# pierrenodet/spark-ensemble

Measured on AMD Instinct MI355X. Metric: rows/sec (whole node) GBMClassifier 100 trees depth=8 at 1/2/4/8 MI355X, higher is better.
Workload: dtype fp32; 1 GPU; model=GBMClassifier(bernoulli, 265 trees, depth=8, bins=256), global_batch=10000000, rows_per_gpu=10000000, features=256, parallelism=dp1

## Files before the change

### csrc/common.h

```cpp
#pragma once

#include <torch/extension.h>
#include <hip/hip_runtime.h>

#include <cstdint>

#define CHECK_GPU(x) TORCH_CHECK(x.is_cuda(), #x " must be on GPU")
#define CHECK_CONTIG(x) TORCH_CHECK(x.is_contiguous(), #x " must be contiguous")

inline int64_t ceil_div(int64_t a, int64_t b) { return (a + b - 1) / b; }

__device__ inline unsigned f32_sortable(float f) {
  unsigned u = __float_as_uint(f);
  return (u & 0x80000000u) ? ~u : (u | 0x80000000u);
}
__device__ inline float sortable_f32(unsigned s) {
  unsigned u = (s & 0x80000000u) ? (s & 0x7FFFFFFFu) : ~s;
  return __uint_as_float(u);
}

enum UploadSlot : int {
  kSlotHistChunks = 0,
  kSlotHistNodes = 1,
  kSlotPartCursors = 2,
  kSlotPartChunks = 3,
  kSlotPartSegStart = 4,
  kSlotGatherSegs = 5,
  kSlotLeafSegs = kSlotGatherSegs,
  kSlotLeafTree = 6,
  kSlotLeafVal = 7,
  kSlotClassChunks = 8,
  kSlotClassNodes = 9,
  kUploadSlots = 12,
};

torch::Tensor h2d_async(const void* src, size_t bytes, UploadSlot slot,
                        const torch::Device& dev);

void launch_hist_decode(float* out, const long long* stage, const int* nodes,
                        const float* scales, int n_multi, int64_t FBC, int C,
                        hipStream_t stream);

void split_argmax_wide(torch::Tensor gain, torch::Tensor feat,
                       torch::Tensor bin, torch::Tensor left_stats,
                       torch::Tensor hist, int D, double lam,
                       double min_child_weight, double min_instances,
                       double min_info_gain);
int64_t hist_build_class(torch::Tensor out, torch::Tensor bins,
                         torch::Tensor bins_t, torch::Tensor label,
                         torch::Tensor weight, torch::Tensor row_idx,
                         torch::Tensor node_offsets, torch::Tensor node_col0,
                         int64_t num_bins, int64_t num_classes, int64_t nn,
                         double w_max, bool identity_rows);

void forest_contrib(torch::Tensor out, torch::Tensor x, torch::Tensor ranges,
                    torch::Tensor path_off, torch::Tensor path_m,
                    torch::Tensor path_v, torch::Tensor e_feat,
                    torch::Tensor e_lo, torch::Tensor e_hi, torch::Tensor e_z,
                    int64_t rows_per_tile, double scale);

void logreg_loss_grad(torch::Tensor payload, torch::Tensor x, torch::Tensor y,
                      torch::Tensor w, torch::Tensor wmat, bool has_bias);
bool logreg_fused_supported(int64_t F, int64_t K);
```

### csrc/ops.hip

```cpp

#include <ATen/hip/HIPContext.h>

#include <chrono>
#include <cstring>
#include <tuple>
#include <vector>

#include "common.h"
#include "hist_plan.h"

torch::Tensor h2d_async(const void* src, size_t bytes, UploadSlot slot,
                        const torch::Device& dev) {
  static thread_local torch::Tensor pin[2 * kUploadSlots];
  static thread_local hipEvent_t done[2 * kUploadSlots] = {};
  static thread_local unsigned char flip[kUploadSlots] = {};
  flip[slot] ^= 1;
  const int bi = slot * 2 + flip[slot];
  auto& b = pin[bi];
  if (done[bi]) (void)hipEventSynchronize(done[bi]);
  if (!b.defined() || (size_t)b.numel() < bytes) {
    size_t cap = 4096;
    while (cap < bytes) cap *= 2;
    b = torch::empty({(int64_t)cap},
                     torch::TensorOptions().dtype(torch::kByte)
// ... 605 lines not shown
    base_l = atomicAdd(cursors + node * 2 + 0, tot);
    base_r = atomicAdd(cursors + node * 2 + 1, -(len - tot)) - (len - tot);
    loc_l = 0;
    loc_r = 0;
  }
  __syncthreads();

  for (int i = threadIdx.x; i < ((len + 63) & ~63); i += blockDim.x) {
    const bool active = i < len;
    const unsigned long long word = bits[i >> 6];
    const bool left = (word >> lane) & 1ull;
    const unsigned long long lmask = word;
    const unsigned long long rmask = __ballot(active) & ~word;
    int lbase = 0, rbase = 0;
    if (lane == 0) {
      lbase = atomicAdd(&loc_l, (int)__popcll(lmask));
      rbase = atomicAdd(&loc_r, (int)__popcll(rmask));
    }
    lbase = __shfl(lbase, 0, 64);
    rbase = __shfl(rbase, 0, 64);
    if (active) {
      const int r = row_idx[start + i];
      if (left) {
        const int pos = base_l + lbase + (int)__popcll(lmask & ((1ull << lane) - 1ull));
        new_rows[pos] = r;
      } else {
        const int pos = base_r + rbase + (int)__popcll(rmask & ((1ull << lane) - 1ull));
        new_rows[pos] = r;
      }
    }
  }
}

void partition_rows(torch::Tensor new_rows, torch::Tensor left_counts,
                    torch::Tensor bins, torch::Tensor bins_t,
                    torch::Tensor row_idx,
                    torch::Tensor node_offsets, torch::Tensor feat,
                    torch::Tensor thr) {
  auto tpA = std::chrono::steady_clock::now();
  CHECK_GPU(new_rows); CHECK_GPU(bins); CHECK_GPU(row_idx);
  CHECK_GPU(feat); CHECK_GPU(thr); CHECK_GPU(left_counts);
  const int F = (int)bins.size(1);
  const int n_nodes = (int)node_offsets.numel() - 1;
  auto offs = node_offsets.accessor<int64_t, 1>();

  std::vector<int> cur_v(n_nodes * 2);
  std::vector<int> chunk_v;
  int64_t total_rows = offs[n_nodes];
  int64_t chunk_rows =
      std::max<int64_t>(8192, ceil_div(total_rows, (int64_t)2048));
  chunk_rows = std::min<int64_t>(chunk_rows, 65536);
  for (int nd = 0; nd < n_nodes; ++nd) {
    cur_v[nd * 2 + 0] = (int)offs[nd];
    cur_v[nd * 2 + 1] = (int)offs[nd + 1];
    for (int64_t c = offs[nd]; c < offs[nd + 1]; c += chunk_rows) {
      chunk_v.push_back(nd);
      chunk_v.push_back((int)c);
      chunk_v.push_back((int)std::min<int64_t>(chunk_rows, offs[nd + 1] - c));
    }
  }
  auto stream = at::hip::getCurrentHIPStream();
  static const bool part_dbg = getenv("SEA_PART_DEBUG") != nullptr;
  auto tp0 = std::chrono::steady_clock::now();
  auto cursors_b = h2d_async(cur_v.data(), cur_v.size() * 4,
                             kSlotPartCursors, bins.device());
  auto cursors = cursors_b.view(torch::kInt32);
  auto tp1 = std::chrono::steady_clock::now();
  if (!chunk_v.empty()) {
    auto chunks_b = h2d_async(chunk_v.data(), chunk_v.size() * 4, kSlotPartChunks,
                              bins.device());
    auto chunks = chunks_b.view(torch::kInt32);
    auto tp2 = std::chrono::steady_clock::now();
    const int n_chunks = (int)(chunk_v.size() / 3);
    const size_t bit_lds = (size_t)((chunk_rows + 63) / 64) * 8;
    const uint8_t* bt_ptr =
        bins_t.defined() && bins_t.numel() ? bins_t.data_ptr<uint8_t>()
                                           : nullptr;
    hipLaunchKernelGGL(partition_kernel, dim3(n_chunks), dim3(256), bit_lds,
                       stream,
                       new_rows.data_ptr<int>(), cursors.data_ptr<int>(),
                       bins.data_ptr<uint8_t>(), bt_ptr,
                       row_idx.data_ptr<int>(),
                       chunks.data_ptr<int>(), feat.data_ptr<int>(),
                       thr.data_ptr<int>(), F, (long long)bins.size(0));
    if (part_dbg) {
      auto tp3 = std::chrono::steady_clock::now();
      auto us = [](auto a, auto b) {
        return std::chrono::duration_cast<std::chrono::microseconds>(b - a)
            .count();
      };
      fprintf(stderr,
              "[part c++] entry=%ldus cursors=%ldus chunks=%ldus launch=%ldus\n",
              (long)us(tpA, tp0), (long)us(tp0, tp1), (long)us(tp1, tp2),
              (long)us(tp2, tp3));
    }
  }
  auto lcur = cursors.view({n_nodes, 2}).select(1, 0);
  std::vector<int> seg_v(n_nodes);
  for (int nd = 0; nd < n_nodes; ++nd) seg_v[nd] = (int)offs[nd];
  auto seg_b = h2d_async(seg_v.data(), seg_v.size() * 4, kSlotPartSegStart,
                         bins.device());
  auto seg_start = seg_b.view(torch::kInt32);
  left_counts.copy_(lcur - seg_start);
}


__global__ void tree_predict_kernel(float* __restrict__ out,
                                    const float* __restrict__ x,
                                    const int* __restrict__ feat,
                                    const float* __restrict__ thr,
                                    const int* __restrict__ left,
                                    const float* __restrict__ leaf,
                                    int64_t n, int F, int D) {
  int64_t i = blockIdx.x * (int64_t)blockDim.x + threadIdx.x;
  int64_t stride = gridDim.x * (int64_t)blockDim.x;
  for (; i < n; i += stride) {
    const float* xr = x + i * F;
    int node = 0;
    int f = feat[0];
    while (f >= 0) {
      node = left[node] + (xr[f] <= thr[node] ? 0 : 1);
      f = feat[node];
    }
    const float* lv = leaf + (int64_t)node * D;
    float* o = out + i * D;
    for (int d = 0; d < D; ++d) o[d] = lv[d];
  }
}

void tree_predict(torch::Tensor out, torch::Tensor x, torch::Tensor feat,
                  torch::Tensor thr, torch::Tensor left, torch::Tensor leaf) {
  CHECK_GPU(out); CHECK_GPU(x);
  int64_t n = x.size(0);
  int F = (int)x.size(1);
  int D = (int)leaf.size(1);
  auto stream = at::hip::getCurrentHIPStream();
// ... 699 lines not shown
  TORCH_CHECK(!want_hess || D == 1, "hessian accumulation is scalar-only");
  TORCH_CHECK(payload.numel() >= 1 + D + (want_hess ? 1 : 0), "payload size");
  auto stream = at::hip::getCurrentHIPStream();
  int blocks = (int)std::min<int64_t>(ceil_div(n, 256 * 8), 2048);
  const int width = 2 + D;
  auto partials = torch::empty({(int64_t)blocks * width},
                               payload.options());
#define LS_LAUNCH(DD)                                                         \
  hipLaunchKernelGGL(line_search_eval_kernel<DD>, dim3(blocks), dim3(256), 0, \
                     stream, partials.data_ptr<float>(),                      \
                     label.data_ptr<float>(), pred.data_ptr<float>(),         \
                     dir.data_ptr<float>(), weight.data_ptr<float>(),         \
                     coeff.data_ptr<float>(), n, (int)loss_id, (float)param,  \
                     want_hess ? 1 : 0)
  switch (D) {
    case 1: LS_LAUNCH(1); break;
    case 2: LS_LAUNCH(2); break;
    case 3: LS_LAUNCH(3); break;
    case 4: LS_LAUNCH(4); break;
    case 5: LS_LAUNCH(5); break;
    case 6: LS_LAUNCH(6); break;
    case 7: LS_LAUNCH(7); break;
    case 8: LS_LAUNCH(8); break;
  }
#undef LS_LAUNCH
  const int rthreads = (256 / width) * width;
  hipLaunchKernelGGL(ls_reduce_kernel, dim3(1), dim3(rthreads), 0, stream,
                     payload.data_ptr<float>(), partials.data_ptr<float>(),
                     blocks, width, std::min(width, (int)payload.numel()));
}


template <int C>
__global__ void split_argmax_kernel(
    unsigned long long* __restrict__ best,
    const float* __restrict__ hist,
    int F, int B, int D, float lam, float min_child_weight,
    float min_instances) {
  const int node = blockIdx.x;
  const int f = blockIdx.y * (blockDim.x >> 6) + (threadIdx.x >> 6);
  const int lane = threadIdx.x & 63;
  if (f >= F) return;
  const float* h = hist + (((int64_t)node * F + f) * (int64_t)B) * C;
  const int BPL = (B + 63) >> 6;
  const int idx_c = C - 1;

  float loc[4][C];
  float tot[C];
#pragma unroll
  for (int c = 0; c < C; ++c) tot[c] = 0.0f;
  for (int i = 0; i < BPL; ++i) {
    const int b = lane * BPL + i;
#pragma unroll
    for (int c = 0; c < C; ++c) loc[i][c] = 0.0f;
    if (b < B) {
#pragma unroll
      for (int c = 0; c < C; ++c) {
        loc[i][c] = h[(int64_t)b * C + c];
        tot[c] += loc[i][c];
      }
    }
  }
  float pre[C], parent[C];
#pragma unroll
  for (int c = 0; c < C; ++c) {
    float v = tot[c];
    for (int off = 1; off < 64; off <<= 1) {
      const float u = __shfl_up(v, off, 64);
      if (lane >= off) v += u;
    }
    pre[c] = v - tot[c];
    parent[c] = __shfl(v, 63, 64);
  }
  float pg2 = 0.0f;
#pragma unroll
  for (int d = 0; d < C; ++d)
    if (d < D) pg2 += parent[d] * parent[d];
  const float parent_score = pg2 / (parent[D] + lam);

  float run[C];
#pragma unroll
  for (int c = 0; c < C; ++c) run[c] = pre[c];
  unsigned best_s = 0u;
  int best_b = -1;
  for (int i = 0; i < BPL; ++i) {
    const int b = lane * BPL + i;
    if (b >= B) break;
#pragma unroll
    for (int c = 0; c < C; ++c) run[c] += loc[i][c];
    if (b < B - 1) {
      const float hl = run[D], hr = parent[D] - run[D];
      const float cl = run[idx_c], cr = parent[idx_c] - run[idx_c];
      if (hl >= min_child_weight && hr >= min_child_weight &&
          cl >= min_instances && cr >= min_instances) {
        float gl = 0.0f, gr = 0.0f;
#pragma unroll
        for (int d = 0; d < C; ++d)
          if (d < D) {
            const float l = run[d], r = parent[d] - run[d];
            gl += l * l;
            gr += r * r;
          }
        const float gain =
            gl / (hl + lam) + gr / (hr + lam) - parent_score;
        const unsigned s = f32_sortable(gain);
        if (s > best_s) { best_s = s; best_b = b; }
      }
    }
  }
  for (int off = 32; off > 0; off >>= 1) {
    const unsigned os = __shfl_down(best_s, off, 64);
    const int ob = __shfl_down(best_b, off, 64);
    if (os > best_s) { best_s = os; best_b = ob; }
  }
  if (lane == 0 && best_b >= 0) {
    const unsigned long long packed =
        ((unsigned long long)best_s << 32) | (unsigned)(f * B + best_b);
    atomicMax(&best[node], packed);
  }
}

template <int C>
__global__ void split_decode_kernel(
    float* __restrict__ gain, int* __restrict__ feat, int* __restrict__ bin,
    float* __restrict__ left_stats,
    const unsigned long long* __restrict__ best,
    const float* __restrict__ hist, int F, int B, float min_info_gain) {
  const int node = blockIdx.x;
  const unsigned long long p = best[node];
  const float g = sortable_f32((unsigned)(p >> 32));
  __shared__ float acc[C];
  if (threadIdx.x < C) acc[threadIdx.x] = 0.0f;
  __syncthreads();
  if (p == 0ull || !(g >= min_info_gain)) {
    if (threadIdx.x == 0) {
      gain[node] = -INFINITY;
      feat[node] = -1;
      bin[node] = -1;
    }
    if (threadIdx.x < C) left_stats[node * C + threadIdx.x] = 0.0f;
    return;
  }
  const int fb = (int)(p & 0xFFFFFFFFull);
  const int f = fb / B, b = fb % B;
  const float* h = hist + (((int64_t)node * F + f) * (int64_t)B) * C;
  float part[C];
#pragma unroll
  for (int c = 0; c < C; ++c) part[c] = 0.0f;
  for (int i = threadIdx.x; i <= b; i += blockDim.x)
#pragma unroll
    for (int c = 0; c < C; ++c) part[c] += h[(int64_t)i * C + c];
#pragma unroll
  for (int c = 0; c < C; ++c)
    if (part[c] != 0.0f) atomicAdd(&acc[c], part[c]);
  __syncthreads();
  if (threadIdx.x == 0) {
    gain[node] = g;
    feat[node] = f;
    bin[node] = b;
  }
  if (threadIdx.x < C) left_stats[node * C + threadIdx.x] = acc[threadIdx.x];
}

void split_argmax(torch::Tensor gain, torch::Tensor feat, torch::Tensor bin,
                  torch::Tensor left_stats, torch::Tensor hist, int64_t d_dims,
                  double lam, double min_child_weight, double min_instances,
                  double min_info_gain) {
  CHECK_GPU(hist); CHECK_CONTIG(hist);
  const int n = (int)hist.size(0);
  const int F = (int)hist.size(1);
  const int B = (int)hist.size(2);
  const int C = (int)hist.size(3);
  const int D = d_dims > 0 ? (int)d_dims : C - 2;
  TORCH_CHECK(C >= 2 && C <= 34, "split_argmax: 2 <= C <= 34");
  TORCH_CHECK(B >= 2 && B <= 256, "split_argmax: 2 <= B <= 256");
  TORCH_CHECK(D >= 1 && D < C, "split_argmax: bad D");
  if (C > 8) {
    CHECK_GPU(gain); CHECK_GPU(feat); CHECK_GPU(bin); CHECK_GPU(left_stats);
    split_argmax_wide(gain, feat, bin, left_stats, hist, D, lam,
                      min_child_weight, min_instances, min_info_gain);
    return;
  }
  auto best = torch::zeros({n}, hist.options().dtype(torch::kInt64));
  auto stream = at::hip::getCurrentHIPStream();
  const int fpb = 4;
#define SA_LAUNCH(CC)                                                         \
  do {                                                                        \
    hipLaunchKernelGGL(split_argmax_kernel<CC>,                               \
                       dim3(n, (F + fpb - 1) / fpb), dim3(64 * fpb), 0,       \
                       stream,                                                \
                       (unsigned long long*)best.data_ptr<int64_t>(),         \
                       hist.data_ptr<float>(), F, B, D, (float)lam,           \
                       (float)min_child_weight, (float)min_instances);        \
    hipLaunchKernelGGL(split_decode_kernel<CC>, dim3(n), dim3(64), 0, stream, \
                       gain.data_ptr<float>(), feat.data_ptr<int>(),          \
                       bin.data_ptr<int>(), left_stats.data_ptr<float>(),     \
                       (unsigned long long*)best.data_ptr<int64_t>(),         \
                       hist.data_ptr<float>(), F, B, (float)min_info_gain);   \
  } while (0)
  switch (C) {
    case 2: SA_LAUNCH(2); break;
    case 3: SA_LAUNCH(3); break;
    case 4: SA_LAUNCH(4); break;
    case 5: SA_LAUNCH(5); break;
    case 6: SA_LAUNCH(6); break;
    case 7: SA_LAUNCH(7); break;
    case 8: SA_LAUNCH(8); break;
  }
#undef SA_LAUNCH
}

std::tuple<int64_t, torch::Tensor, torch::Tensor> hist_plan_debug(
    torch::Tensor node_offsets, torch::Tensor node_col0, int64_t row_bound,
    int64_t col_bound, int64_t lds_bytes, int64_t n_groups) {
  auto offs = node_offsets.to(torch::kInt64).contiguous();
  auto col0 = node_col0.to(torch::kInt32).contiguous();
  const int n_nodes = (int)offs.numel() - 1;
  TORCH_CHECK(col0.numel() == 0 || col0.numel() == n_nodes,
              "node_col0 must be empty or have one entry per node");
  HistPlan plan = plan_hist_chunks(
      offs.data_ptr<int64_t>(), n_nodes,
      col0.numel() ? col0.data_ptr<int>() : nullptr, row_bound,
      (int)col_bound, (size_t)lds_bytes, (int)n_groups, 0);
  auto i32 = torch::TensorOptions().dtype(torch::kInt32);
  auto chunks = torch::tensor(plan.table, i32).view({plan.n_chunks, 5});
  auto multi = torch::tensor(plan.multi_nodes, i32);
  return {plan.chunk_rows, chunks, multi};
}

std::tuple<torch::Tensor, torch::Tensor> hist_plan_slots_debug(
    torch::Tensor node_offsets, torch::Tensor node_col0, int64_t row_bound,
    int64_t col_bound, int64_t lds_bytes, int64_t n_groups) {
  auto offs = node_offsets.to(torch::kInt64).contiguous();
  auto col0 = node_col0.to(torch::kInt32).contiguous();
  const int n_nodes = (int)offs.numel() - 1;
  TORCH_CHECK(col0.numel() == 0 || col0.numel() == n_nodes,
              "node_col0 must be empty or have one entry per node");
  HistPlan plan = plan_hist_chunks(
      offs.data_ptr<int64_t>(), n_nodes,
      col0.numel() ? col0.data_ptr<int>() : nullptr, row_bound,
      (int)col_bound, (size_t)lds_bytes, (int)n_groups, 0);
  auto i32 = torch::TensorOptions().dtype(torch::kInt32);
  return {torch::tensor(plan.slot_first, i32),
          torch::tensor(plan.slot_count, i32)};
}

PYBIND11_MODULE(TORCH_EXTENSION_NAME, m) {
  m.def("_hist_plan", &hist_plan_debug,
        "host-side chunk plan of the histogram kernels (no device)");
  m.def("_hist_plan_slots", &hist_plan_slots_debug,
        "first record and record count of each staging slot of _hist_plan");
  m.def("gather_ranges_gh", &gather_ranges_gh,
        "gather_ranges plus the compact gh rows of the gathered rows");
  m.def("logreg_loss_grad", &logreg_loss_grad,
        "single-pass fused logistic loss+gradient");
  m.def("logreg_fused_supported", &logreg_fused_supported);
  m.def("split_argmax", &split_argmax,
        "fused best-split gain scan + argmax over node histograms");
  m.def("sample_weights", &sample_weights, "counter-based Poisson/Bernoulli row weights");
  m.def("bin_features", &bin_features, "quantile binning f32 -> u8");
  m.def("hist_build", &hist_build, "LDS-staged node histograms",
        py::arg("out"), py::arg("bins"), py::arg("gh"), py::arg("row_idx"),
        py::arg("node_offsets"), py::arg("num_bins"), py::arg("d_dims"),
        py::arg("max_abs"), py::arg("identity_rows"), py::arg("node_col0"),
        py::arg("c_per_node"), py::arg("gh_by_position") = false);
  m.def("hist_build_class", &hist_build_class,
        "label-indexed node histograms for K-class gini trees");
  m.def("partition_rows", &partition_rows, "block-aggregated node partition");
  m.def("tree_predict", &tree_predict, "single-tree batched predict");
  m.def("forest_predict", &forest_predict, "packed-forest weighted predict");
  m.def("forest_predict2", &forest_predict2,
        "LDS-staged tree-group-tiled forest predict");
  m.def("forest_contrib", &forest_contrib,
        "per-row feature contributions (TreeSHAP) of a packed forest");
  m.def("transpose_u8", &transpose_u8, "tiled u8 matrix transpose");
  m.def("gather_ranges", &gather_ranges,
        "one-pass concat of contiguous index ranges");
  m.def("leaf_scatter", &leaf_scatter,
        "scatter per-segment leaf values into the [N, T] train-pred matrix");
  m.def("grad_hess", &grad_hess, "fused per-row loss gradient/hessian");
  m.def("line_search_eval", &line_search_eval, "fused loss+grad line-search payload");
  m.def("newton_chain_1d", &newton_chain_1d,
        "device-chained safeguarded-Newton stage-weight search");
}
```

### spark_ensemble_amd/models/tree_grower.py

```python

from __future__ import annotations

from dataclasses import dataclass
from typing import Dict, List, Optional, Tuple

import torch

from ..ops import dispatch as ops
from ..parallel import Comm


@dataclass
class GrowParams:
    max_depth: int = 5
    max_bins: int = 32
    min_instances_per_node: int = 1
    min_info_gain: float = 0.0
    min_child_weight: float = 0.0
    lam: float = 1e-6


def ensure_binned(frame, x: torch.Tensor, max_bins: int):
    cached = frame.cache_get("bins", x, max_bins) if frame is not None else None
    if cached is not None:
# ... 580 lines not shown
        cnt_col = torch.tensor([float(v) for v in root_lens], device=device)
    if root_tot_in is None:
        cols = [g_sum, h_sum.unsqueeze(1)]
        if NN == 2:
            cols.append(cnt_col.unsqueeze(1))
        root_tot = torch.cat(cols, dim=1)
        if comm is not None:
            comm.all_reduce_(root_tot)
        totals = root_tot.cpu()

    covers_t[:, 0] = totals[:, D]

    node_tree = torch.arange(T, dtype=torch.long)
    node_nid = torch.zeros(T, dtype=torch.long)
    off_acc = [0]
    for v in root_lens:
        off_acc.append(off_acc[-1] + v)
    offsets = torch.tensor(off_acc, dtype=torch.int64)
    hists: Optional[torch.Tensor] = None
    parent_of_t: Optional[torch.Tensor] = None
    built_mask_t: Optional[torch.Tensor] = None

    edges_cpu = edges.cpu()
    idx_c = C - 1

    capture = train_pred_out is not None and D == 1
    tp_arena = (
        torch.zeros(N, T, dtype=torch.float32, device=device)
        if capture else None
    )

    pending_writes = None

    def _finalize_and_capture(idx_t, offs, ridx):
        if idx_t.numel() == 0:
            return
        t_ids = node_tree[idx_t]
        nids = node_nid[idx_t]
        g = totals[idx_t, :D]
        h = totals[idx_t, D]
        denom = (h + params.lam).unsqueeze(1)
        vals = torch.where(denom > 0, g / denom, torch.zeros_like(g))
        leaves_t[t_ids, nids] = vals
        if capture:
            starts = offs[idx_t]
            lens = offs[idx_t + 1] - starts
            nz = (lens > 0).nonzero(as_tuple=True)[0]
            if nz.numel():
                ops.leaf_scatter(tp_arena, ridx, starts[nz], lens[nz],
                                 t_ids[nz], vals[nz, 0])

    for depth in range(params.max_depth + 1):
        n_active = int(node_tree.numel())
        if n_active == 0:
            break
        if depth == params.max_depth:
            _finalize_and_capture(torch.arange(n_active), offsets, row_idx)
            break

        split_args = dict(
            lam=params.lam,
            min_child_weight=params.min_child_weight,
            min_instances=params.min_instances_per_node,
            min_info_gain=params.min_info_gain,
            d_dims=D,
        )
        lvl_mask = None
        if feature_masks is not None:
            lvl_mask = feature_masks.index_select(
                0, _to_dev_async(node_tree, device)
            )
        if hists is None:
            if class_mode:
                new_h = _class_hist(row_idx, offsets, node_tree,
                                    identity=(root_rows is None and T == 1))
            else:
                new_h = ops.hist_build_forest(
                    bins, gh, row_idx, offsets,
                    (node_tree * C).to(torch.int32), B, C, gh_max, d_dims=D,
                )
            hists, gain, feat, b, left_stats = _finish_level_split(
                new_h, None, None, None, None, None, n_active, (F, B, C),
                device, comm, split_args, split_mask=lvl_mask,
            )
        else:
            built_cpu = built_mask_t.nonzero(as_tuple=True)[0]
            nb_cpu = (~built_mask_t).nonzero(as_tuple=True)[0]
            bh = None
            if built_cpu.numel():
                starts = offsets[built_cpu]
                lens = offsets[built_cpu + 1] - starts
                b_off = torch.zeros(built_cpu.numel() + 1, dtype=torch.int64)
                b_off[1:] = torch.cumsum(lens, 0)
                if class_mode:
                    build_rows = ops.gather_ranges(row_idx, starts, lens)
                    bh = _class_hist(build_rows, b_off, node_tree[built_cpu])
                else:
                    build_rows, gh_b = ops.gather_ranges_gh(
                        row_idx, gh, starts, lens, node_tree[built_cpu] * C,
                        C,
                    )
                    bh = ops.hist_build_forest(
                        bins, gh_b, build_rows, b_off,
                        torch.zeros(built_cpu.numel(), dtype=torch.int32),
                        B, C, gh_max, d_dims=D, gh_by_position=True,
                    )
            hists, gain, feat, b, left_stats = _finish_level_split(
                bh, _to_dev_async(built_cpu, device), hists,
                _to_dev_async(nb_cpu, device),
                _to_dev_async(nb_cpu ^ 1, device),
                _to_dev_async(parent_of_t[nb_cpu], device), n_active,
                (F, B, C), device, comm, split_args, split_mask=lvl_mask,
            )
        pack_d = torch.cat([
            gain, feat.to(torch.float32), b.to(torch.float32),
            left_stats.reshape(-1),
        ])
        ev = None
        if bins.is_cuda:
            pack_h = torch.empty(pack_d.numel(), dtype=torch.float32,
                                 pin_memory=True)
            pack_h.copy_(pack_d, non_blocking=True)
            ev = torch.cuda.Event()
            ev.record()

        pr_async = None
        if bins.is_cuda:
            pr_async = ops.partition_rows_async(bins, row_idx, offsets, feat, b)

        if pending_writes is not None:
            pending_writes()
            pending_writes = None

        if ev is not None:
            ev.synchronize()
            pack = pack_h
        else:
            pack = pack_d
        gain_cpu = pack[:n_active]
        feat_cpu = pack[n_active:2 * n_active].to(torch.int32)
        b_cpu = pack[2 * n_active:3 * n_active].to(torch.int32)
        left_stats = pack[3 * n_active:].reshape(n_active, C)

        do_split = torch.isfinite(gain_cpu)
        ns_idx = (~do_split).nonzero(as_tuple=True)[0]
        _finalize_and_capture(ns_idx, offsets, row_idx)
        if not bool(do_split.any()):
            break

        s_idx = do_split.nonzero(as_tuple=True)[0]
        t_ids = node_tree[s_idx]
        nids = node_nid[s_idx]
        f_l = feat_cpu[s_idx].long()
        b_l = b_cpu[s_idx].long()
        counts = torch.bincount(t_ids, minlength=T)
        firsts = torch.cumsum(counts, 0) - counts
        rank = torch.arange(s_idx.numel(), dtype=torch.long) - firsts[t_ids]
        cid = cur_len[t_ids] + 2 * rank
        cur_len += 2 * counts

        hists = hists.index_select(0, _to_dev_async(s_idx, device))

        l_st = left_stats[s_idx]
        r_st = totals[s_idx] - l_st
        totals = torch.stack([l_st, r_st], dim=1).reshape(-1, C)
        l_cnt = l_st[:, idx_c]
        r_cnt = r_st[:, idx_c]
        built_mask_t = torch.stack([l_cnt <= r_cnt, l_cnt > r_cnt],
                                   dim=1).reshape(-1)
        parent_of_t = torch.arange(s_idx.numel(),
                                   dtype=torch.long).repeat_interleave(2)
        node_tree = t_ids.repeat_interleave(2)
        node_nid = torch.stack([cid, cid + 1], dim=1).reshape(-1)

        def _writes(t_ids=t_ids, nids=nids, f_l=f_l, b_l=b_l,
                    gains=gain_cpu[s_idx].double(), cid=cid,
                    l_cov=l_st[:, D], r_cov=r_st[:, D]):
            feats_t[t_ids, nids] = f_l.to(torch.int32)
            thrs_t[t_ids, nids] = edges_cpu[f_l, b_l]
            fi.index_put_((t_ids, f_l), gains, accumulate=True)
            lefts_t[t_ids, nids] = cid.to(torch.int32)
            covers_t[t_ids, cid] = l_cov
            covers_t[t_ids, cid + 1] = r_cov
        pending_writes = _writes

        if pr_async is not None:
            new_rows, new_offs, _ = ops.partition_rows_finish(*pr_async)
        else:
            split_feat = torch.where(do_split, feat_cpu,
                                     torch.full_like(feat_cpu, -1))
            new_rows, new_offs, _ = ops.partition_rows(
                bins, row_idx, offsets,
                split_feat.to(torch.int32), b_cpu.to(torch.int32),
            )
# ... 48 lines not shown
```

### spark_ensemble_amd/ops/dispatch.py

```python

from __future__ import annotations

import math
import os
from typing import Optional

import torch

from . import reference

_hip = None
_hip_error: Optional[str] = None


def _load_hip():
    global _hip, _hip_error
    if _hip is not None or _hip_error is not None:
        return _hip
    try:
        from . import hip_ext

        _hip = hip_ext.load()
    except Exception as e:
        _hip_error = f"{type(e).__name__}: {e}"
# ... 80 lines not shown
                    )
                    parts.append(part[..., :w])
                    if ci == len(spans) - 1:
                        parts.append(part[..., w:])
                return torch.cat(parts, dim=-1)
            return _hist_build_launch(
                m, bins, gh, row_idx, node_offsets, _EMPTY_I32, num_bins, C,
                max_abs, d_dims, identity_rows,
            )
    return reference.hist_build(bins, gh, row_idx, node_offsets, num_bins)


_EMPTY_I32 = torch.empty(0, dtype=torch.int32)
_EMPTY_U8 = torch.empty(0, dtype=torch.uint8)


def _hist_build_launch(m, bins, gh, row_idx, node_offsets, node_col0,
                       num_bins, c_per_node, max_abs, d_dims, identity_rows,
                       gh_by_position=False):
    out = torch.empty(
        node_offsets.numel() - 1, bins.shape[1], num_bins, c_per_node,
        dtype=torch.float32, device=bins.device,
    )
    m.hist_build(
        out, bins, gh.contiguous(), row_idx.to(torch.int32),
        node_offsets.to(torch.int64).cpu().contiguous(), int(num_bins),
        int(d_dims), max_abs.to(torch.float32), bool(identity_rows),
        node_col0, int(c_per_node), bool(gh_by_position),
    )
    return out


def hist_build_forest(bins, gh, row_idx, node_offsets, node_col0, num_bins,
                      c_per_node, max_abs, d_dims=1, gh_by_position=False):
    if bins.is_cuda:
        m = _require_hip("hist_build")
        if m is not None:
            return _hist_build_launch(
                m, bins, gh, row_idx, node_offsets,
                node_col0.to(torch.int32).cpu().contiguous(), num_bins,
                c_per_node, max_abs, d_dims, False, gh_by_position,
            )
    if gh_by_position:
        pos = torch.arange(row_idx.numel(), device=row_idx.device)
        return reference.hist_build_forest(
            bins.index_select(0, row_idx.long()), gh, pos, node_offsets,
            node_col0, num_bins, c_per_node
        )
    return reference.hist_build_forest(
        bins, gh, row_idx, node_offsets, node_col0, num_bins, c_per_node
    )


last_hist_build_class_info: dict = {}


def hist_build_class(bins, label, weight, row_idx, node_offsets, node_col0,
                     num_bins, num_classes, nn, w_max=None,
                     identity_rows=False, transposed=None):
    if bins.is_cuda:
        m = _require_hip("hist_build_class")
        if m is not None:
            n_nodes = node_offsets.numel() - 1
            F = bins.shape[1]
            C = int(num_classes) + int(nn)
            if w_max is None:
                w_max = float(weight.max()) if weight.numel() else 1.0
            if transposed is None:
                transposed = os.environ.get("SEA_CLASS_HIST_SRC") != "rowmajor"
            bt = _bins_transposed(bins) if transposed else _EMPTY_U8
            out = torch.empty(n_nodes, F, num_bins, C, dtype=torch.float32,
                              device=bins.device)
            n_multi = m.hist_build_class(
                out, bins, bt, label, weight.contiguous(),
# ... 8 lines not shown
    return reference.hist_build_class(
        bins, label, weight, row_idx, node_offsets, node_col0, num_bins,
        num_classes, nn,
    )


SPLIT_WIDE_MAX_C = 34


def split_search(hist, lam=1e-6, min_child_weight=0.0, min_instances=1.0, min_info_gain=0.0, d_dims=-1):
    if hist.is_cuda:
        c_chk = hist.shape[3]
        if c_chk > SPLIT_WIDE_MAX_C:
            return reference.split_search(
                hist, lam, min_child_weight, min_instances, min_info_gain,
                d_dims,
            )
        m = _require_hip("split_argmax")
        if m is not None:
            n, f, b, c = hist.shape
            gain = torch.empty(n, dtype=torch.float32, device=hist.device)
            feat = torch.empty(n, dtype=torch.int32, device=hist.device)
            bin_ = torch.empty(n, dtype=torch.int32, device=hist.device)
            left_stats = torch.empty(n, c, dtype=torch.float32, device=hist.device)
            m.split_argmax(
                gain, feat, bin_, left_stats, hist.contiguous(),
                int(d_dims), float(lam), float(min_child_weight),
                float(min_instances), float(min_info_gain),
            )
            return gain, feat.long(), bin_.long(), left_stats
    return reference.split_search(hist, lam, min_child_weight, min_instances, min_info_gain, d_dims)


def partition_rows(bins, row_idx, node_offsets, feat, thr):
    if bins.is_cuda:
        m = _require_hip("partition_rows")
        if m is not None:
            new_rows, lc_dev, offs_cpu = partition_rows_async(
                bins, row_idx, node_offsets, feat, thr
            )
            return partition_rows_finish(new_rows, lc_dev, offs_cpu)
    return reference.partition_rows(bins, row_idx, node_offsets, feat, thr)


_BT_CACHE: list = []


def _bins_transposed(bins):
    import weakref

    m = _load_hip()
    if m is None or not bins.is_cuda:
        return None
    _BT_CACHE[:] = [(w, b) for (w, b) in _BT_CACHE if w() is not None]
    for wr, bt in _BT_CACHE:
        if wr() is bins:
            return bt
    n, f = bins.shape
    bt = torch.empty(f, n, dtype=torch.uint8, device=bins.device)
    m.transpose_u8(bt, bins)
    _BT_CACHE.insert(0, (weakref.ref(bins), bt))
    del _BT_CACHE[1:]
    return bt


def partition_rows_async(bins, row_idx, node_offsets, feat, thr):
    import time as _time

    _prof = os.environ.get("SEA_GROW_PROF") == "1"
    _t0 = _time.perf_counter() if _prof else 0.0
    m = _require_hip("partition_rows")
    n = node_offsets.numel() - 1
    offs_cpu = node_offsets.to(torch.int64).cpu()
    row_idx = row_idx.to(torch.int32)
    new_rows = torch.empty_like(row_idx)
    left_counts = torch.zeros(n, dtype=torch.int32, device=bins.device)
    f32 = feat.to(torch.int32).to(bins.device)
    t32 = thr.to(torch.int32).to(bins.device)
    if _prof:
        _t1 = _time.perf_counter()
    bt = _bins_transposed(bins)
    m.partition_rows(
        new_rows,
        left_counts,
        bins,
        bt if bt is not None else _EMPTY_U8,
        row_idx,
        offs_cpu,
        f32,
        t32,
    )
    lc_h = torch.empty(left_counts.numel(), dtype=torch.int32,
                       pin_memory=True)
    lc_h.copy_(left_counts, non_blocking=True)
    ev = torch.cuda.Event()
    ev.record()
    if _prof:
        _t2 = _time.perf_counter()
        print(f"[part prof] prep={(_t1-_t0)*1000:.2f} native={(_t2-_t1)*1000:.2f}")
    return new_rows, (lc_h, ev), offs_cpu


def gather_ranges(src, starts, lens):
    if src.is_cuda:
        m = _require_hip("gather_ranges")
        if m is not None:
            out = torch.empty(int(lens.sum()), dtype=torch.int32,
                              device=src.device)
            m.gather_ranges(out, src, starts.to(torch.int64),
                            lens.to(torch.int64))
            return out
    st, ln = starts.tolist(), lens.tolist()
    segs = [src[s:s + l] for s, l in zip(st, ln) if l > 0]
    if not segs:
# ... 15 lines not shown
                               col0.to(torch.int64))
            return out, gh_out
    rows = gather_ranges(src, starts, lens)
    segs = [
        gh[src[s:s + l].long(), c0:c0 + C]
        for s, l, c0 in zip(starts.tolist(), lens.tolist(), col0.tolist())
        if l > 0
    ]
    if not segs:
        return rows, gh.new_empty(0, C)
    return rows, torch.cat(segs)


def leaf_scatter(tp, row_idx, starts, lens, tree, val):
    if tp.is_cuda:
        m = _require_hip("leaf_scatter")
        if m is not None:
            m.leaf_scatter(tp, row_idx, starts.to(torch.int64),
                           lens.to(torch.int64), tree.to(torch.int64),
                           val.to(torch.float32))
            return
    st, ln = starts.tolist(), lens.tolist()
    tl, vl = tree.tolist(), val.tolist()
    for s, l, t, v in zip(st, ln, tl, vl):
        if l > 0:
            tp[row_idx[s:s + l].long(), int(t)] = float(v)


def partition_rows_finish(new_rows, left_counts, offs_cpu):
    n = offs_cpu.numel() - 1
    if isinstance(left_counts, tuple):
        lc_h, ev = left_counts
        ev.synchronize()
        lc = lc_h.to(torch.int64)
    else:
        lc = left_counts.cpu().to(torch.int64)
    sizes = torch.empty(2 * n, dtype=torch.int64)
    seg = offs_cpu[1:] - offs_cpu[:-1]
    sizes[0::2] = lc
    sizes[1::2] = seg - lc
    new_offs = torch.cat([torch.zeros(1, dtype=torch.int64), sizes.cumsum(0)])
    return new_rows, new_offs, lc


def tree_predict(x, feature, threshold, left_child, leaf_value, max_depth):
    if x.is_cuda:
        m = _require_hip("tree_predict")
        if m is not None:
            N = x.shape[0]
            D = leaf_value.shape[1]
            out = torch.empty(N, D, dtype=torch.float32, device=x.device)
            m.tree_predict(
                out,
                x.contiguous(),
                feature.to(torch.int32).to(x.device),
                threshold.to(torch.float32).to(x.device),
                left_child.to(torch.int32).to(x.device),
                leaf_value.to(torch.float32).to(x.device).contiguous(),
            )
            return out
    return reference.tree_predict(x, feature, threshold, left_child, leaf_value, max_depth)


def forest_predict(x, trees, weights=None, max_depth=64, cache=None):
    if x.is_cuda and trees:
        m = _require_hip("forest_predict")
        if m is not None:
# ... 325 lines not shown
```

Baseline: 1.219 billion rows/sec.

## Fuse sibling-subtraction, level histogram assembly and split search into one kernel

Adds a level_split op whose kernel builds each node's histogram (copying built rows or computing parent minus sibling), optionally stores it, and runs the split scan in one pass, then decodes straight into a packed result buffer. This replaces the gather/subtract/index_select steps, the separate split search and the torch.cat packing with fewer launches and fewer passes over the histograms. Partition also returns raw cursors copied to pinned host memory, so the device-side left-count subtraction kernel and its upload disappear. The cost is a host-side table build per level and heavier validation on the host.

```diff
diff --git a/csrc/common.h b/csrc/common.h
--- a/csrc/common.h
+++ b/csrc/common.h
@@ -31,6 +31,7 @@
   kSlotLeafVal = 7,
   kSlotClassChunks = 8,
   kSlotClassNodes = 9,
+  kSlotLevelTable = 10,
   kUploadSlots = 12,
 };
 
diff --git a/csrc/ops.hip b/csrc/ops.hip
--- a/csrc/ops.hip
+++ b/csrc/ops.hip
@@ -661,14 +661,14 @@
   }
 }
 
-void partition_rows(torch::Tensor new_rows, torch::Tensor left_counts,
-                    torch::Tensor bins, torch::Tensor bins_t,
-                    torch::Tensor row_idx,
-                    torch::Tensor node_offsets, torch::Tensor feat,
-                    torch::Tensor thr) {
+static torch::Tensor partition_launch(torch::Tensor new_rows,
+                                      torch::Tensor bins, torch::Tensor bins_t,
+                                      torch::Tensor row_idx,
+                                      torch::Tensor node_offsets,
+                                      torch::Tensor feat, torch::Tensor thr) {
   auto tpA = std::chrono::steady_clock::now();
   CHECK_GPU(new_rows); CHECK_GPU(bins); CHECK_GPU(row_idx);
-  CHECK_GPU(feat); CHECK_GPU(thr); CHECK_GPU(left_counts);
+  CHECK_GPU(feat); CHECK_GPU(thr);
   const int F = (int)bins.size(1);
   const int n_nodes = (int)node_offsets.numel() - 1;
   auto offs = node_offsets.accessor<int64_t, 1>();
@@ -724,13 +724,44 @@
               (long)us(tp2, tp3));
     }
   }
-  auto lcur = cursors.view({n_nodes, 2}).select(1, 0);
+  return cursors.view({n_nodes, 2});
+}
+
+void partition_rows(torch::Tensor new_rows, torch::Tensor left_counts,
+                    torch::Tensor bins, torch::Tensor bins_t,
+                    torch::Tensor row_idx,
+                    torch::Tensor node_offsets, torch::Tensor feat,
+                    torch::Tensor thr) {
+  CHECK_GPU(left_counts);
+  auto cursors = partition_launch(new_rows, bins, bins_t, row_idx,
+                                  node_offsets, feat, thr);
+  const int n_nodes = (int)node_offsets.numel() - 1;
+  auto offs = node_offsets.accessor<int64_t, 1>();
+  auto lcur = cursors.select(1, 0);
   std::vector<int> seg_v(n_nodes);
   for (int nd = 0; nd < n_nodes; ++nd) seg_v[nd] = (int)offs[nd];
   auto seg_b = h2d_async(seg_v.data(), seg_v.size() * 4, kSlotPartSegStart,
                          bins.device());
   auto seg_start = seg_b.view(torch::kInt32);
   left_counts.copy_(lcur - seg_start);
+}
+
+torch::Tensor partition_rows_cursors(torch::Tensor new_rows,
+                                     torch::Tensor bins, torch::Tensor bins_t,
+                                     torch::Tensor row_idx,
+                                     torch::Tensor node_offsets,
+                                     torch::Tensor feat, torch::Tensor thr) {
+  CHECK_CONTIG(new_rows); CHECK_CONTIG(row_idx); CHECK_CONTIG(feat);
+  CHECK_CONTIG(thr);
+  const int64_t n_nodes = node_offsets.numel() - 1;
+  TORCH_CHECK(feat.scalar_type() == torch::kInt32 &&
+                  thr.scalar_type() == torch::kInt32 &&
+                  feat.numel() == n_nodes && thr.numel() == n_nodes,
+              "partition_rows_cursors: feat and thr are int32 [n_nodes]");
+  TORCH_CHECK(new_rows.numel() == row_idx.numel(),
+              "partition_rows_cursors: new_rows must match row_idx");
+  return partition_launch(new_rows, bins, bins_t, row_idx, node_offsets, feat,
+                          thr);
 }
 
 
@@ -1496,6 +1527,72 @@
 
 
 template <int C>
+__device__ __forceinline__ void split_scan_wave(
+    unsigned long long* __restrict__ best, float (&loc)[4][C], float (&tot)[C],
+    int node, int f, int lane, int B, int D, float lam,
+    float min_child_weight, float min_instances) {
+  const int BPL = (B + 63) >> 6;
+  const int idx_c = C - 1;
+  float pre[C], parent[C];
+#pragma unroll
+  for (int c = 0; c < C; ++c) {
+    float v = tot[c];
+    for (int off = 1; off < 64; off <<= 1) {
+      const float u = __shfl_up(v, off, 64);
+      if (lane >= off) v += u;
+    }
+    pre[c] = v - tot[c];
+    parent[c] = __shfl(v, 63, 64);
+  }
+  float pg2 = 0.0f;
+#pragma unroll
+  for (int d = 0; d < C; ++d)
+    if (d < D) pg2 += parent[d] * parent[d];
+  const float parent_score = pg2 / (parent[D] + lam);
+
+  float run[C];
+#pragma unroll
+  for (int c = 0; c < C; ++c) run[c] = pre[c];
+  unsigned best_s = 0u;
+  int best_b = -1;
+  for (int i = 0; i < BPL; ++i) {
+    const int b = lane * BPL + i;
+    if (b >= B) break;
+#pragma unroll
+    for (int c = 0; c < C; ++c) run[c] += loc[i][c];
+    if (b < B - 1) {
+      const float hl = run[D], hr = parent[D] - run[D];
+      const float cl = run[idx_c], cr = parent[idx_c] - run[idx_c];
+      if (hl >= min_child_weight && hr >= min_child_weight &&
+          cl >= min_instances && cr >= min_instances) {
+        float gl = 0.0f, gr = 0.0f;
+#pragma unroll
+        for (int d = 0; d < C; ++d)
+          if (d < D) {
+            const float l = run[d], r = parent[d] - run[d];
+            gl += l * l;
+            gr += r * r;
+          }
+        const float gain =
+            gl / (hl + lam) + gr / (hr + lam) - parent_score;
+        const unsigned s = f32_sortable(gain);
+        if (s > best_s) { best_s = s; best_b = b; }
+      }
+    }
+  }
+  for (int off = 32; off > 0; off >>= 1) {
+    const unsigned os = __shfl_down(best_s, off, 64);
+    const int ob = __shfl_down(best_b, off, 64);
+    if (os > best_s) { best_s = os; best_b = ob; }
+  }
+  if (lane == 0 && best_b >= 0) {
+    const unsigned long long packed =
+        ((unsigned long long)best_s << 32) | (unsigned)(f * B + best_b);
+    atomicMax(&best[node], packed);
+  }
+}
+
+template <int C>
 __global__ void split_argmax_kernel(
     unsigned long long* __restrict__ best,
     const float* __restrict__ hist,
@@ -1507,7 +1604,6 @@
   if (f >= F) return;
   const float* h = hist + (((int64_t)node * F + f) * (int64_t)B) * C;
   const int BPL = (B + 63) >> 6;
-  const int idx_c = C - 1;
 
   float loc[4][C];
   float tot[C];
@@ -1525,66 +1621,57 @@
       }
     }
   }
-  float pre[C], parent[C];
-#pragma unroll
-  for (int c = 0; c < C; ++c) {
-    float v = tot[c];
-    for (int off = 1; off < 64; off <<= 1) {
-      const float u = __shfl_up(v, off, 64);
-      if (lane >= off) v += u;
-    }
-    pre[c] = v - tot[c];
-    parent[c] = __shfl(v, 63, 64);
-  }
-  float pg2 = 0.0f;
-#pragma unroll
-  for (int d = 0; d < C; ++d)
-    if (d < D) pg2 += parent[d] * parent[d];
-  const float parent_score = pg2 / (parent[D] + lam);
-
-  float run[C];
-#pragma unroll
-  for (int c = 0; c < C; ++c) run[c] = pre[c];
-  unsigned best_s = 0u;
-  int best_b = -1;
+  split_scan_wave<C>(best, loc, tot, node, f, lane, B, D, lam,
+                     min_child_weight, min_instances);
+}
+
+template <int C>
+__global__ void level_scan_kernel(
+    unsigned long long* __restrict__ best,
+    float* level,
+    const float* built,
+    const float* __restrict__ parent,
+    const int* __restrict__ tab,
+    int store, int F, int B, int D, float lam, float min_child_weight,
+    float min_instances) {
+  const int node = blockIdx.x;
+  const int f = blockIdx.y * (blockDim.x >> 6) + (threadIdx.x >> 6);
+  const int lane = threadIdx.x & 63;
+  if (f >= F) return;
+  const int b_row = tab[node * 3 + 0];
+  const int64_t slice = (int64_t)B * C;
+  const float* h = built + ((int64_t)(b_row >= 0 ? b_row : tab[node * 3 + 2]) *
+                                F + f) * slice;
+  const float* ph =
+      b_row >= 0 ? nullptr
+                 : parent + ((int64_t)tab[node * 3 + 1] * F + f) * slice;
+  float* o = level + ((int64_t)node * F + f) * slice;
+  const int BPL = (B + 63) >> 6;
+
+  float loc[4][C];
+  float tot[C];
+#pragma unroll
+  for (int c = 0; c < C; ++c) tot[c] = 0.0f;
   for (int i = 0; i < BPL; ++i) {
     const int b = lane * BPL + i;
-    if (b >= B) break;
-#pragma unroll
-    for (int c = 0; c < C; ++c) run[c] += loc[i][c];
-    if (b < B - 1) {
-      const float hl = run[D], hr = parent[D] - run[D];
-      const float cl = run[idx_c], cr = parent[idx_c] - run[idx_c];
-      if (hl >= min_child_weight && hr >= min_child_weight &&
-          cl >= min_instances && cr >= min_instances) {
-        float gl = 0.0f, gr = 0.0f;
-#pragma unroll
-        for (int d = 0; d < C; ++d)
-          if (d < D) {
-            const float l = run[d], r = parent[d] - run[d];
-            gl += l * l;
-            gr += r * r;
-          }
-        const float gain =
-            gl / (hl + lam) + gr / (hr + lam) - parent_score;
-        const unsigned s = f32_sortable(gain);
-        if (s > best_s) { best_s = s; best_b = b; }
-      }
-    }
-  }
-  for (int off = 32; off > 0; off >>= 1) {
-    const unsigned os = __shfl_down(best_s, off, 64);
-    const int ob = __shfl_down(best_b, off, 64);
-    if (os > best_s) { best_s = os; best_b = ob; }
-  }
-  if (lane == 0 && best_b >= 0) {
-    const unsigned long long packed =
-        ((unsigned long long)best_s << 32) | (unsigned)(f * B + best_b);
-    atomicMax(&best[node], packed);
-  }
-}
-
-template <int C>
+#pragma unroll
+    for (int c = 0; c < C; ++c) loc[i][c] = 0.0f;
+    if (b < B) {
+#pragma unroll
+      for (int c = 0; c < C; ++c) {
+        float v = h[(int64_t)b * C + c];
+        if (ph) v = ph[(int64_t)b * C + c] - v;
+        if (store) o[(int64_t)b * C + c] = v;
+        loc[i][c] = v;
+        tot[c] += loc[i][c];
+      }
+    }
+  }
+  split_scan_wave<C>(best, loc, tot, node, f, lane, B, D, lam,
+                     min_child_weight, min_instances);
+}
+
+template <int C, bool PACK = false>
 __global__ void split_decode_kernel(
     float* __restrict__ gain, int* __restrict__ feat, int* __restrict__ bin,
     float* __restrict__ left_stats,
@@ -1601,6 +1688,10 @@
       gain[node] = -INFINITY;
       feat[node] = -1;
       bin[node] = -1;
+      if (PACK) {
+        gain[gridDim.x + node] = -1.0f;
+        gain[2 * gridDim.x + node] = -1.0f;
+      }
     }
     if (threadIdx.x < C) left_stats[node * C + threadIdx.x] = 0.0f;
     return;
@@ -1622,6 +1713,10 @@
     gain[node] = g;
     feat[node] = f;
     bin[node] = b;
+    if (PACK) {
+      gain[gridDim.x + node] = (float)f;
+      gain[2 * gridDim.x + node] = (float)b;
+    }
   }
   if (threadIdx.x < C) left_stats[node * C + threadIdx.x] = acc[threadIdx.x];
 }
@@ -1674,6 +1769,135 @@
 #undef SA_LAUNCH
 }
 
+void level_split(torch::Tensor level, torch::Tensor pack, torch::Tensor feat,
+                 torch::Tensor bin, torch::Tensor built, torch::Tensor parent,
+                 torch::Tensor table, int64_t d_dims, double lam,
+                 double min_child_weight, double min_instances,
+                 double min_info_gain) {
+  CHECK_GPU(level); CHECK_GPU(pack); CHECK_GPU(feat); CHECK_GPU(bin);
+  CHECK_GPU(built);
+  CHECK_CONTIG(level); CHECK_CONTIG(pack); CHECK_CONTIG(feat);
+  CHECK_CONTIG(bin); CHECK_CONTIG(built); CHECK_CONTIG(parent);
+  CHECK_CONTIG(table);
+  TORCH_CHECK(!table.is_cuda() && table.scalar_type() == torch::kInt32 &&
+                  table.dim() == 2 && table.size(1) == 3,
+              "level_split: table must be a host int32 [n, 3]");
+  TORCH_CHECK(level.dim() == 4 && built.dim() == 4,
+              "level_split: level and built must be [n, F, B, C]");
+  TORCH_CHECK(level.scalar_type() == torch::kFloat32 &&
+                  built.scalar_type() == torch::kFloat32 &&
+                  pack.scalar_type() == torch::kFloat32 &&
+                  feat.scalar_type() == torch::kInt32 &&
+                  bin.scalar_type() == torch::kInt32,
+              "level_split: f32 histograms and pack, int32 feat and bin");
+  const int64_t n = level.size(0);
+  const int64_t n_built = built.size(0);
+  const int F = (int)level.size(1);
+  const int B = (int)level.size(2);
+  const int C = (int)level.size(3);
+  const int D = d_dims > 0 ? (int)d_dims : C - 2;
+  TORCH_CHECK(built.size(1) == F && built.size(2) == B && built.size(3) == C,
+              "level_split: built and level disagree in F, B, C");
+  const bool has_parent = parent.numel() > 0;
+  int64_t n_prev = 0;
+  if (has_parent) {
+    CHECK_GPU(parent);
+    TORCH_CHECK(parent.dim() == 4 && parent.scalar_type() == torch::kFloat32 &&
+                    parent.size(1) == F && parent.size(2) == B &&
+                    parent.size(3) == C,
+                "level_split: parent and level disagree in F, B, C");
+    n_prev = parent.size(0);
+    TORCH_CHECK(parent.data_ptr() != level.data_ptr(),
+                "level_split: level must not be parent");
+  }
+  TORCH_CHECK(level.device() == built.device() &&
+                  pack.device() == built.device() &&
+                  feat.device() == built.device() &&
+                  bin.device() == built.device() &&
+                  (!has_parent || parent.device() == built.device()),
+              "level_split: all device tensors on one device");
+  TORCH_CHECK(n < ((int64_t)1 << 31), "level_split: too many nodes");
+  TORCH_CHECK(C >= 2 && C <= 8, "level_split: 2 <= C <= 8");
+  TORCH_CHECK(B >= 2 && B <= 256, "level_split: 2 <= B <= 256");
+  TORCH_CHECK(D >= 1 && D < C, "level_split: bad D");
+  TORCH_CHECK(table.size(0) == n, "level_split: one table row per node");
+  TORCH_CHECK(pack.numel() == n * (3 + C) && feat.numel() == n &&
+                  bin.numel() == n,
+              "level_split: pack is [n * (3 + C)], feat and bin are [n]");
+  const bool alias = level.data_ptr() == built.data_ptr();
+  TORCH_CHECK(!alias || n == n_built,
+              "level_split: level may alias built only when every node is "
+              "built in place");
+  auto overlaps = [](const torch::Tensor& a, const torch::Tensor& b) {
+    const char* a0 = (const char*)a.data_ptr();
+    const char* b0 = (const char*)b.data_ptr();
+    return a0 < b0 + b.nbytes() && b0 < a0 + a.nbytes();
+  };
+  TORCH_CHECK(alias || !overlaps(level, built),
+              "level_split: level overlaps built without being it");
+  TORCH_CHECK(!has_parent || !overlaps(level, parent),
+              "level_split: level overlaps parent");
+  auto tb = table.accessor<int, 2>();
+  for (int64_t j = 0; j < n; ++j) {
+    const int br = tb[j][0];
+    if (br >= 0) {
+      TORCH_CHECK(br < n_built, "level_split: built_row ", br, " of node ", j,
+                  " out of range");
+      TORCH_CHECK(!alias || br == j,
+                  "level_split: level aliases built but node ", j,
+                  " is built in row ", br);
+      continue;
+    }
+    TORCH_CHECK(br == -1, "level_split: built_row of node ", j, " is ", br);
+    TORCH_CHECK(!alias, "level_split: level aliases built but node ", j,
+                " is derived");
+    TORCH_CHECK(tb[j][1] >= 0 && tb[j][1] < n_prev,
+                "level_split: parent_row ", tb[j][1], " of node ", j,
+                " out of range");
+    TORCH_CHECK(tb[j][2] >= 0 && tb[j][2] < n_built,
+                "level_split: sibling_built_row ", tb[j][2], " of node ", j,
+                " out of range");
+    const int64_t sib = j ^ 1;
+    TORCH_CHECK(sib < n && tb[sib][0] == tb[j][2],
+                "level_split: the sibling of derived node ", j,
+                " is not the built node in row ", tb[j][2]);
+  }
+  if (n == 0 || F == 0) return;
+  auto tab = h2d_async(table.data_ptr(), (size_t)n * 12, kSlotLevelTable,
+                       level.device());
+  auto best = torch::zeros({n}, level.options().dtype(torch::kInt64));
+  auto stream = at::hip::getCurrentHIPStream();
+  const int fpb = 4;
+  float* pk = pack.data_ptr<float>();
+#define LS_LAUNCH(CC)                                                         \
+  do {                                                                        \
+    hipLaunchKernelGGL(level_scan_kernel<CC>,                                 \
+                       dim3((unsigned)n, (F + fpb - 1) / fpb),                \
+                       dim3(64 * fpb), 0, stream,                             \
+                       (unsigned long long*)best.data_ptr<int64_t>(),         \
+                       level.data_ptr<float>(), built.data_ptr<float>(),      \
+                       has_parent ? parent.data_ptr<float>() : nullptr,       \
+                       (const int*)tab.data_ptr(), alias ? 0 : 1, F, B, D,    \
+                       (float)lam, (float)min_child_weight,                   \
+                       (float)min_instances);                                 \
+    hipLaunchKernelGGL((split_decode_kernel<CC, true>), dim3((unsigned)n),    \
+                       dim3(64), 0, stream, pk, feat.data_ptr<int>(),         \
+                       bin.data_ptr<int>(), pk + 3 * n,                       \
+                       (unsigned long long*)best.data_ptr<int64_t>(),         \
+                       level.data_ptr<float>(), F, B, (float)min_info_gain);  \
+  } while (0)
+  switch (C) {
+    case 2: LS_LAUNCH(2); break;
+    case 3: LS_LAUNCH(3); break;
+    case 4: LS_LAUNCH(4); break;
+    case 5: LS_LAUNCH(5); break;
+    case 6: LS_LAUNCH(6); break;
+    case 7: LS_LAUNCH(7); break;
+    case 8: LS_LAUNCH(8); break;
+  }
+#undef LS_LAUNCH
+}
+
 std::tuple<int64_t, torch::Tensor, torch::Tensor> hist_plan_debug(
     torch::Tensor node_offsets, torch::Tensor node_col0, int64_t row_bound,
     int64_t col_bound, int64_t lds_bytes, int64_t n_groups) {
@@ -1731,6 +1955,10 @@
   m.def("hist_build_class", &hist_build_class,
         "label-indexed node histograms for K-class gini trees");
   m.def("partition_rows", &partition_rows, "block-aggregated node partition");
+  m.def("partition_rows_cursors", &partition_rows_cursors,
+        "node partition that returns its cursor table");
+  m.def("level_split", &level_split,
+        "split search of one tree level on built / parent - sibling in place");
   m.def("tree_predict", &tree_predict, "single-tree batched predict");
   m.def("forest_predict", &forest_predict, "packed-forest weighted predict");
   m.def("forest_predict2", &forest_predict2,
diff --git a/spark_ensemble_amd/models/tree_grower.py b/spark_ensemble_amd/models/tree_grower.py
--- a/spark_ensemble_amd/models/tree_grower.py
+++ b/spark_ensemble_amd/models/tree_grower.py
@@ -636,6 +636,13 @@
 
     pending_writes = None
 
+    fused = (
+        bins.is_cuda and C <= 8 and feature_masks is None
+        and not (comm is not None and comm.is_distributed and F >= 32)
+        and ops.level_fused_enabled()
+    )
+    parent_row_t: Optional[torch.Tensor] = None
+
     def _finalize_and_capture(idx_t, offs, ridx):
         if idx_t.numel() == 0:
             return
@@ -682,11 +689,20 @@
                 new_h = ops.hist_build_forest(
                     bins, gh, row_idx, offsets,
                     (node_tree * C).to(torch.int32), B, C, gh_max, d_dims=D,
+                    identity_rows=(fused and root_rows is None and T == 1),
                 )
-            hists, gain, feat, b, left_stats = _finish_level_split(
-                new_h, None, None, None, None, None, n_active, (F, B, C),
-                device, comm, split_args, split_mask=lvl_mask,
-            )
+            if fused:
+                if comm is not None:
+                    comm.all_reduce_(new_h)
+                table = torch.full((n_active, 3), -1, dtype=torch.int32)
+                table[:, 0] = torch.arange(n_active, dtype=torch.int32)
+                hists, pack_d, feat, b = ops.level_split(
+                    new_h, None, table, **split_args)
+            else:
+                hists, gain, feat, b, left_stats = _finish_level_split(
+                    new_h, None, None, None, None, None, n_active, (F, B, C),
+                    device, comm, split_args, split_mask=lvl_mask,
+                )
         else:
             built_cpu = built_mask_t.nonzero(as_tuple=True)[0]
             nb_cpu = (~built_mask_t).nonzero(as_tuple=True)[0]
@@ -709,17 +725,30 @@
                         torch.zeros(built_cpu.numel(), dtype=torch.int32),
                         B, C, gh_max, d_dims=D, gh_by_position=True,
                     )
-            hists, gain, feat, b, left_stats = _finish_level_split(
-                bh, _to_dev_async(built_cpu, device), hists,
-                _to_dev_async(nb_cpu, device),
-                _to_dev_async(nb_cpu ^ 1, device),
-                _to_dev_async(parent_of_t[nb_cpu], device), n_active,
-                (F, B, C), device, comm, split_args, split_mask=lvl_mask,
-            )
-        pack_d = torch.cat([
-            gain, feat.to(torch.float32), b.to(torch.float32),
-            left_stats.reshape(-1),
-        ])
+            if fused:
+                if comm is not None:
+                    comm.all_reduce_(bh)
+                brow = torch.full((n_active,), -1, dtype=torch.long)
+                brow[built_cpu] = torch.arange(built_cpu.numel())
+                table = torch.full((n_active, 3), -1, dtype=torch.int32)
+                table[:, 0] = brow
+                table[nb_cpu, 1] = parent_row_t[nb_cpu].to(torch.int32)
+                table[nb_cpu, 2] = brow[nb_cpu ^ 1].to(torch.int32)
+                hists, pack_d, feat, b = ops.level_split(
+                    bh, hists, table, **split_args)
+            else:
+                hists, gain, feat, b, left_stats = _finish_level_split(
+                    bh, _to_dev_async(built_cpu, device), hists,
+                    _to_dev_async(nb_cpu, device),
+                    _to_dev_async(nb_cpu ^ 1, device),
+                    _to_dev_async(parent_of_t[nb_cpu], device), n_active,
+                    (F, B, C), device, comm, split_args, split_mask=lvl_mask,
+                )
+        if not fused:
+            pack_d = torch.cat([
+                gain, feat.to(torch.float32), b.to(torch.float32),
+                left_stats.reshape(-1),
+            ])
         ev = None
         if bins.is_cuda:
             pack_h = torch.empty(pack_d.numel(), dtype=torch.float32,
@@ -763,7 +792,10 @@
         cid = cur_len[t_ids] + 2 * rank
         cur_len += 2 * counts
 
-        hists = hists.index_select(0, _to_dev_async(s_idx, device))
+        if fused:
+            parent_row_t = s_idx.repeat_interleave(2)
+        else:
+            hists = hists.index_select(0, _to_dev_async(s_idx, device))
 
         l_st = left_stats[s_idx]
         r_st = totals[s_idx] - l_st
diff --git a/spark_ensemble_amd/ops/dispatch.py b/spark_ensemble_amd/ops/dispatch.py
--- a/spark_ensemble_amd/ops/dispatch.py
+++ b/spark_ensemble_amd/ops/dispatch.py
@@ -136,14 +136,16 @@
 
 
 def hist_build_forest(bins, gh, row_idx, node_offsets, node_col0, num_bins,
-                      c_per_node, max_abs, d_dims=1, gh_by_position=False):
+                      c_per_node, max_abs, d_dims=1, gh_by_position=False,
+                      identity_rows=False):
     if bins.is_cuda:
         m = _require_hip("hist_build")
         if m is not None:
             return _hist_build_launch(
                 m, bins, gh, row_idx, node_offsets,
                 node_col0.to(torch.int32).cpu().contiguous(), num_bins,
-                c_per_node, max_abs, d_dims, False, gh_by_position,
+                c_per_node, max_abs, d_dims, bool(identity_rows),
+                gh_by_position,
             )
     if gh_by_position:
         pos = torch.arange(row_idx.numel(), device=row_idx.device)
@@ -218,6 +220,82 @@
     return reference.split_search(hist, lam, min_child_weight, min_instances, min_info_gain, d_dims)
 
 
+def level_fused_enabled() -> bool:
+    return os.environ.get("SEA_LEVEL_FUSED", "1") != "0"
+
+
+def _check_level_table(table, n_built, n_prev):
+    tb = table.tolist()
+    n = len(tb)
+    for j, (br, pr, sr) in enumerate(tb):
+        if br >= 0:
+            if br >= n_built:
+                raise RuntimeError(f"level_split: built_row {br} of node {j} "
+                                   "out of range")
+            continue
+        if br != -1:
+            raise RuntimeError(f"level_split: built_row of node {j} is {br}")
+        if not 0 <= pr < n_prev:
+            raise RuntimeError(f"level_split: parent_row {pr} of node {j} "
+                               "out of range")
+        if not 0 <= sr < n_built:
+            raise RuntimeError(f"level_split: sibling_built_row {sr} of node "
+                               f"{j} out of range")
+        if (j ^ 1) >= n or tb[j ^ 1][0] != sr:
+            raise RuntimeError(f"level_split: the sibling of derived node {j} "
+                               f"is not the built node in row {sr}")
+
+
+def level_split(built, parent, table, lam=1e-6, min_child_weight=0.0,
+                min_instances=1.0, min_info_gain=0.0, d_dims=-1):
+    table = table.to(torch.int32).cpu().contiguous()
+    n = table.shape[0]
+    n_built, F, B, C = built.shape
+    root = parent is None or parent.numel() == 0
+    n_prev = 0 if root else parent.shape[0]
+    if not root and tuple(parent.shape[1:]) != (F, B, C):
+        raise RuntimeError("level_split: parent and built disagree in F, B, C")
+    identity = n == n_built and bool(
+        (table[:, 0] == torch.arange(n, dtype=torch.int32)).all())
+    args = (float(lam), float(min_child_weight), float(min_instances),
+            float(min_info_gain))
+    if built.is_cuda and C <= 8 and level_fused_enabled():
+        m = _require_hip("level_split")
+        if m is not None:
+            dev = built.device
+            built = built.contiguous()
+            level = built if root and identity else torch.empty(
+                n, F, B, C, dtype=torch.float32, device=dev)
+            pack = torch.empty(n * (3 + C), dtype=torch.float32, device=dev)
+            feat = torch.empty(n, dtype=torch.int32, device=dev)
+            bin_ = torch.empty(n, dtype=torch.int32, device=dev)
+            m.level_split(
+                level, pack, feat, bin_, built,
+                built.new_empty(0) if root else parent.contiguous(), table,
+                int(d_dims), *args,
+            )
+            return level, pack, feat, bin_
+    _check_level_table(table, n_built, n_prev)
+    dev = built.device
+    if root and identity:
+        level = built
+    else:
+        tb = table.long()
+        b_nodes = (tb[:, 0] >= 0).nonzero(as_tuple=True)[0]
+        d_nodes = (tb[:, 0] < 0).nonzero(as_tuple=True)[0]
+        level = torch.empty(n, F, B, C, dtype=torch.float32, device=dev)
+        if b_nodes.numel():
+            level[b_nodes.to(dev)] = built[tb[b_nodes, 0].to(dev)]
+        if d_nodes.numel():
+            level[d_nodes.to(dev)] = (
+                parent[tb[d_nodes, 1].to(dev)] - built[tb[d_nodes, 2].to(dev)]
+            )
+    g, ft, b, ls = split_search(level, *args, d_dims=d_dims)
+    pack = torch.cat([g, ft.to(torch.float32), b.to(torch.float32),
+                      ls.reshape(-1)])
+    return level, pack, ft.to(torch.int32), b.to(torch.int32)
+
+
 def partition_rows(bins, row_idx, node_offsets, feat, thr):
     if bins.is_cuda:
         m = _require_hip("partition_rows")
@@ -260,12 +338,23 @@
     offs_cpu = node_offsets.to(torch.int64).cpu()
     row_idx = row_idx.to(torch.int32)
     new_rows = torch.empty_like(row_idx)
-    left_counts = torch.zeros(n, dtype=torch.int32, device=bins.device)
     f32 = feat.to(torch.int32).to(bins.device)
     t32 = thr.to(torch.int32).to(bins.device)
+    bt = _bins_transposed(bins)
+    if level_fused_enabled():
+        cursors = m.partition_rows_cursors(
+            new_rows, bins, bt if bt is not None else _EMPTY_U8,
+            row_idx.contiguous(), offs_cpu, f32.contiguous(),
+            t32.contiguous(),
+        )
+        cur_h = torch.empty(n, 2, dtype=torch.int32, pin_memory=True)
+        cur_h.copy_(cursors, non_blocking=True)
+        ev = torch.cuda.Event()
+        ev.record()
+        return new_rows, (cur_h, ev), offs_cpu
+    left_counts = torch.zeros(n, dtype=torch.int32, device=bins.device)
     if _prof:
         _t1 = _time.perf_counter()
-    bt = _bins_transposed(bins)
     m.partition_rows(
         new_rows,
         left_counts,
@@ -347,7 +436,10 @@
     if isinstance(left_counts, tuple):
         lc_h, ev = left_counts
         ev.synchronize()
-        lc = lc_h.to(torch.int64)
+        if lc_h.dim() == 2:
+            lc = lc_h[:, 0].to(torch.int64) - offs_cpu[:-1]
+        else:
+            lc = lc_h.to(torch.int64)
     else:
         lc = left_counts.cpu().to(torch.int64)
     sizes = torch.empty(2 * n, dtype=torch.int64)
```

Result: faster. 1.381 billion rows/sec, median of 6 (+13.3%).
